# DenDen047/AcinoSet

Measured on AMD Instinct MI355X. Metric: frames/sec to SBA convergence, 6-cam x 20-kp (points-only SBA, configs[1]), higher is better.
Workload: dtype f64; 1 GPU; sba_points C=6 frames=100/rank L=20 (configs[1]); n_points_per_rank=2000, obs_slots_per_rank=12000, parallelism=frame-shard x1

## Files before the change

acinoset_amd/_native.py:

```python
from __future__ import annotations

import ctypes as C
import os
import threading
from typing import Optional

import numpy as np

try:
    import torch
except Exception:
    torch = None

_HERE = os.path.dirname(os.path.abspath(__file__))
LIB_PATH = os.environ.get('ACINOSET_HIP_LIB', os.path.join(_HERE, 'libacinoset_hip.so'))

ACS_DEVICE_PTRS = 1
ACS_CAM_STRIDE = 20
STATUS_NAMES = ('running', 'gtol', 'ftol', 'xtol', 'stalled', 'maxiter', 'noobs')
SD_MODES = {'const': 0, 'variable': 1}

SYMBOLS = (
    'acs_ctx_create', 'acs_ctx_destroy', 'acs_last_error', 'acs_ctx_set_stream', 'acs_ctx_sync',
    'acs_abi_version', 'acs_device_count', 'acs_sba_default_opts', 'acs_project_fisheye',
    'acs_sba_residuals', 'acs_sba_points', 'acs_sba_points_dense', 'acs_redescending_loss', 'acs_fk',
    'acs_fte_default_opts', 'acs_fte_solve', 'acs_fte_eval', 'acs_triangulate_pairs', 'acs_triangulate_dense',
    'acs_sba_ext_default_opts', 'acs_sba_extrinsics', 'acs_sba_points_dense_io',
    'acs_fte_dist_create', 'acs_fte_dist_init', 'acs_fte_dist_round', 'acs_fte_dist_poll',
    'acs_fte_dist_gather', 'acs_fte_dist_scatter', 'acs_fte_dist_result',
    'acs_fte_dist_destroy', 'acs_fte_dist_reset', 'acs_alloc_events', 'acs_ekf_singular_count',
    'acs_fte_debug_blocks', 'acs_fte_debug_plan',
    'acs_sba_ext_dist_create', 'acs_sba_ext_dist_init', 'acs_sba_ext_dist_round', 'acs_sba_ext_dist_poll',
    'acs_sba_ext_dist_result', 'acs_sba_ext_dist_destroy', 'acs_ekf_run',
    'acs_sba_ekf_pipeline', 'acs_fte_covariance',
)


class NativeUnavailable(RuntimeError):
    pass


class SbaOpts(C.Structure):
    _fields_ = [('max_iters', C.c_int32), ('reserved', C.c_int32), ('f_scale', C.c_double),
                ('ftol', C.c_double), ('xtol', C.c_double), ('gtol', C.c_double)]


class Report(C.Structure):
    _fields_ = [('n_problems', C.c_int64), ('status_counts', C.c_int64 * 7), ('iters_max', C.c_int64),
                ('iters_sum', C.c_int64), ('nfev_sum', C.c_int64), ('cost_before', C.c_double),
                ('cost_after', C.c_double)]

    def as_dict(self):
        return dict(n_problems=self.n_problems,
                    status_counts={STATUS_NAMES[i]: int(self.status_counts[i]) for i in range(7)},
                    iters_max=self.iters_max, iters_sum=self.iters_sum, nfev_sum=self.nfev_sum,
                    cost_before=self.cost_before, cost_after=self.cost_after)


class EkfInitSpec(C.Structure):
    _fields_ = [(k, C.c_int32) for k in ('nose', 'lure', 'x0', 'y0', 'psi0', 'xl', 'yl', 'from_sba')]


def ekf_numerics_mode(ref_numerics, jacobian):
    if jacobian == 'analytic':
        if ref_numerics:
            raise ValueError("jacobian='analytic' runs in float64: pass ref_numerics=False")
        return 2
# ... 44 lines not shown

    def as_dict(self):
        d = {k: getattr(self, k) for k, _ in self._fields_}
        d['status_name'] = STATUS_NAMES[self.status] if 0 <= self.status < 7 else str(self.status)
        return d


ABI_VERSION = 5
_lib = None
_lock = threading.Lock()
_P = C.c_void_p
_D = C.POINTER(C.c_double)


def _declare(lib):
    i32, i64, u32, dbl = C.c_int32, C.c_int64, C.c_uint32, C.c_double
    sig = {
        'acs_ctx_create': (C.c_int, [C.c_int, C.POINTER(_P)]),
        'acs_ctx_destroy': (C.c_int, [_P]),
        'acs_last_error': (C.c_char_p, [_P]),
        'acs_ctx_set_stream': (C.c_int, [_P, _P]),
        'acs_ctx_sync': (C.c_int, [_P]),
        'acs_abi_version': (C.c_int, []),
        'acs_device_count': (C.c_int, [C.POINTER(C.c_int)]),
        'acs_sba_default_opts': (None, [C.POINTER(SbaOpts)]),
        'acs_project_fisheye': (C.c_int, [_P, _P, i32, _P, _P, i64, i32, _P, u32]),
        'acs_sba_residuals': (C.c_int, [_P, _P, i32, _P, _P, _P, i64, _P, i64, _P, u32]),
        'acs_sba_points': (C.c_int, [_P, _P, i32, _P, _P, _P, i64, _P, i64, C.POINTER(SbaOpts), _P, _P,
                                     C.POINTER(Report), u32]),
        'acs_sba_points_dense': (C.c_int, [_P, _P, i32, _P, _P, i64, _P, C.POINTER(SbaOpts), C.POINTER(Report),
                                           u32]),
        'acs_sba_points_dense_io': (C.c_int, [_P, _P, i32, _P, _P, i64, _P, _P, C.POINTER(SbaOpts),
                                              C.POINTER(Report), u32]),
        'acs_redescending_loss': (C.c_int, [_P, _P, i64, dbl, dbl, dbl, _P, _P, u32]),
        'acs_fk': (C.c_int, [_P, _P, i64, _P, i64, _P, _P, _P, _P, i64, i32, i32, _P, _P, u32]),
        'acs_fte_default_opts': (None, [C.POINTER(FteOpts)]),
        'acs_fte_solve': (C.c_int, [_P, _P, i64, _P, i64, _P, i32, _P, _P, i32, i32, dbl, _P, i32, i32, _P, _P,
                                    C.POINTER(FteOpts), C.POINTER(FteReport), u32]),
        'acs_fte_eval': (C.c_int, [_P, _P, i64, _P, i64, _P, i32, _P, _P, i32, i32, dbl, _P, i32, i32, _P, _P,
                                   _P, _P, _P, u32]),
        'acs_fte_covariance': (C.c_int, [_P, _P, i64, _P, i64, _P, i32, _P, _P, i32, i32, dbl, _P, i32, i32, _P, _P,
                                         _P, _P, _P, C.POINTER(FteCovReport), u32]),
        'acs_fte_debug_blocks': (C.c_int, [_P, _P, i64, _P, i64, _P, i32, _P, _P, i32, i32, dbl, _P, i32, i32, _P, _P,
                                           dbl, i32, _P, C.POINTER(i64), u32]),
        'acs_fte_debug_plan': (C.c_int, [_P, i32, i32, i32, i32, i32, i32, C.POINTER(i32), C.POINTER(i32), i32]),
        'acs_triangulate_pairs': (C.c_int, [_P, _P, i32, _P, _P, _P, _P, i64, _P, u32]),
        'acs_triangulate_dense': (C.c_int, [_P, _P, i32, _P, _P, i64, _P, _P, u32]),
        'acs_sba_ext_default_opts': (None, [C.POINTER(SbaExtOpts)]),
        'acs_fte_dist_create': (C.c_int, [_P, _P, i64, _P, i64, _P, i32, _P, _P, i32, i32, dbl, _P, i32, i32, _P, _P,
                                          C.POINTER(FteOpts), i32, i32, C.POINTER(_P), C.POINTER(i64), u32]),
        'acs_fte_dist_init': (C.c_int, [_P, _P]),
        'acs_fte_dist_round': (C.c_int, [_P, _P, _P]),
        'acs_fte_dist_poll': (C.c_int, [_P, i64, C.POINTER(i32)]),
        'acs_fte_dist_gather': (C.c_int, [_P, _P]),
        'acs_fte_dist_scatter': (C.c_int, [_P, _P]),
        'acs_fte_dist_result': (C.c_int, [_P, _P, _P, C.POINTER(FteReport), u32]),
        'acs_fte_dist_destroy': (C.c_int, [_P]),
        'acs_fte_dist_reset': (C.c_int, [_P, _P, _P, u32]),
        'acs_alloc_events': (C.c_int64, []),
        'acs_ekf_singular_count': (C.c_int, [_P, C.POINTER(i32)]),
        'acs_sba_ext_dist_create': (C.c_int, [_P, _P, i32, _P, _P, _P, i64, _P, i64, C.POINTER(SbaExtOpts), i32, i32,
                                              C.POINTER(_P), C.POINTER(i64), u32]),
        'acs_sba_ext_dist_init': (C.c_int, [_P, _P]),
        'acs_sba_ext_dist_round': (C.c_int, [_P, _P, _P]),
        'acs_sba_ext_dist_poll': (C.c_int, [_P, C.c_int64, C.POINTER(i32)]),
        'acs_sba_ext_dist_result': (C.c_int, [_P, _P, _P, C.POINTER(SbaExtReport), u32]),
# ... 130 lines not shown
                                                int(bool(fte_form)), _ptr(out), 0), 'acs_project_fisheye')
        return out

    def sba_residuals(self, cams, uv, pt_idx, cam_idx, pts):
        cams = _c64(cams)
        uv = _c64(uv).reshape(-1, 2)
        pi = np.ascontiguousarray(pt_idx, np.int32)
        ci = np.ascontiguousarray(cam_idx, np.int32)
        pts = _c64(pts).reshape(-1, 3)
        out = np.empty(2 * len(uv))
        self.check(self.lib.acs_sba_residuals(self.h, _ptr(cams), len(cams), _ptr(uv), _ptr(pi), _ptr(ci), len(uv),
                                              _ptr(pts), len(pts), _ptr(out), 0), 'acs_sba_residuals')
        return out

    @staticmethod
    def sba_opts(f_scale=50.0, max_iters=100, ftol=1e-15, xtol=1e-9, gtol=1e-10):
        return SbaOpts(int(max_iters), 0, float(f_scale), float(ftol), float(xtol), float(gtol))

    def sba_points(self, cams, uv, pt_idx, cam_idx, pts0, opts=None, residuals=True):
        cams = _c64(cams)
        uv = _c64(uv).reshape(-1, 2)
        pi = np.ascontiguousarray(pt_idx, np.int32)
        ci = np.ascontiguousarray(cam_idx, np.int32)
        pts = _c64(pts0).reshape(-1, 3).copy()
        rb = np.empty(2 * len(uv)) if residuals else None
        ra = np.empty(2 * len(uv)) if residuals else None
        rep = Report()
        opts = opts or self.sba_opts()
        self.check(self.lib.acs_sba_points(self.h, _ptr(cams), len(cams), _ptr(uv), _ptr(pi), _ptr(ci), len(uv),
                                           _ptr(pts), len(pts), C.byref(opts), _ptr(rb), _ptr(ra), C.byref(rep), 0),
                   'acs_sba_points')
        return pts, rb, ra, rep.as_dict()

    def sba_points_dense(self, cams, uv, mask, pts0, opts=None):
        cams = _c64(cams)
        C_ = len(cams)
        uv = _c64(uv).reshape(-1, C_, 2)
        mask = np.ascontiguousarray(mask, np.uint8).reshape(-1, C_)
        pts = _c64(pts0).reshape(-1, 3).copy()
        rep = Report()
        opts = opts or self.sba_opts()
        self.check(self.lib.acs_sba_points_dense(self.h, _ptr(cams), C_, _ptr(uv), _ptr(mask), len(pts), _ptr(pts),
                                                 C.byref(opts), C.byref(rep), 0), 'acs_sba_points_dense')
        return pts, rep.as_dict()

    def sba_points_dense_dev(self, cams_p, n_cams, uv_p, mask_p, n_pts, pts_p, opts=None, report=False,
                             pts_in_p=None):
        opts = opts or self.sba_opts()
        rep = Report() if report else None
        rp = C.byref(rep) if rep is not None else None
        if pts_in_p is None:
            rc = self.lib.acs_sba_points_dense(self.h, C.c_void_p(cams_p), n_cams, C.c_void_p(uv_p),
                                               C.c_void_p(mask_p), n_pts, C.c_void_p(pts_p), C.byref(opts), rp,
                                               ACS_DEVICE_PTRS)
        else:
            rc = self.lib.acs_sba_points_dense_io(self.h, C.c_void_p(cams_p), n_cams, C.c_void_p(uv_p),
                                                  C.c_void_p(mask_p), n_pts, C.c_void_p(pts_in_p),
                                                  C.c_void_p(pts_p), C.byref(opts), rp, ACS_DEVICE_PTRS)
        self.check(rc, 'acs_sba_points_dense')
        return rep.as_dict() if rep is not None else None

    def sba_ext_opts(self, **kw):
        o = SbaExtOpts()
        self.lib.acs_sba_ext_default_opts(C.byref(o))
        for k, v in kw.items():
            setattr(o, k, v)
# ... 286 lines not shown
```

acinoset_amd/build.py:

```python
import glob
import os
import subprocess
import sys
from concurrent.futures import ThreadPoolExecutor

HERE = os.path.dirname(os.path.abspath(__file__))
REPO = os.path.dirname(HERE)
CSRC = os.path.join(HERE, 'csrc')
OUT = os.path.join(HERE, 'libacinoset_hip.so')
HIPCC = os.environ.get('HIPCC', '/opt/rocm/bin/hipcc')
ARCH = 'gfx950'
CFLAGS = ['-O3', '-std=c++17', '-fPIC', f'--offload-arch={ARCH}', '-I', os.path.join(REPO, 'include'),
          '-Wno-unused-result']


def _newest(paths):
    return max(os.path.getmtime(p) for p in paths)


def build(force: bool = False, verbose: bool = True, jobs: int = 8) -> str:
    srcs = sorted(glob.glob(os.path.join(CSRC, '*.hip')))
    deps = srcs + glob.glob(os.path.join(CSRC, '*.hpp')) + [os.path.join(REPO, 'include', 'acinoset_hip.h')]
    if not force and os.path.exists(OUT) and os.path.getmtime(OUT) >= _newest(deps):
        return OUT
    objdir = os.path.join(CSRC, 'build')
    os.makedirs(objdir, exist_ok=True)
    hdr_t = _newest([d for d in deps if not d.endswith('.hip')])

    def compile_one(src):
        obj = os.path.join(objdir, os.path.basename(src)[:-4] + '.o')
        if not force and os.path.exists(obj) and os.path.getmtime(obj) >= max(os.path.getmtime(src), hdr_t):
            return obj
        cmd = [HIPCC, *CFLAGS, '-c', src, '-o', obj]
        if verbose:
            print(' '.join(cmd), flush=True)
        subprocess.run(cmd, check=True)
        return obj

    with ThreadPoolExecutor(max_workers=jobs) as ex:
        objs = list(ex.map(compile_one, srcs))
    cmd = [HIPCC, f'--offload-arch={ARCH}', '-shared', '-fPIC', *objs, '-o', OUT]
    if verbose:
        print(' '.join(cmd), flush=True)
    subprocess.run(cmd, check=True)
    return OUT


if __name__ == '__main__':
    build(force='--force' in sys.argv)
```

acinoset_amd/csrc/common.hpp:

```cpp
#pragma once

#include <hip/hip_runtime.h>

#include <cmath>
#include <cstdarg>
#include <cstdint>
#include <cstdio>
#include <cstring>
#include <string>
#include <vector>

#include "acinoset_hip.h"

enum WsSlot {
  WS_CAMS = 0, WS_UV, WS_MASK, WS_CAMID, WS_PTS, WS_PTIDX, WS_CAMIDX, WS_OUT0, WS_OUT1,
  WS_PERPT_F0, WS_PERPT_F1, WS_PERPT_I, WS_REPORT, WS_SORT0, WS_SORT1, WS_SORT2, WS_SORT3,
  WS_TMP0, WS_TMP1, WS_TMP2, WS_TMP3, WS_TMP4, WS_TMP5, WS_TMP6, WS_TMP7,
  WS_FTE0, WS_FTE1, WS_FTE2, WS_FTE3, WS_FTE4, WS_FTE5, WS_FTE6, WS_FTE7, WS_FTE8, WS_FTE9,
  WS_FTE10, WS_FTE11, WS_FTE12, WS_FTE13, WS_FTE14, WS_FTE15,
  WS_PIPE0, WS_PIPE1, WS_PIPE2, WS_PIPE3, WS_PIPE4, WS_PIPE5, WS_PIPE6, WS_PIPE7,
  WS_NSLOTS
};
struct acs_ctx {
  int device = 0;
  hipStream_t own_stream = nullptr;
  hipStream_t stream = nullptr;
  std::string err;
  void* ws[WS_NSLOTS] = {};
  size_t ws_bytes[WS_NSLOTS] = {};
  int n_cu = 256;
  void* pinned = nullptr;
  size_t pinned_bytes = 0;
  int* ekf_bad = nullptr;
  void* fte_cov = nullptr;
  size_t fte_cov_bytes = 0;
};

hipError_t acs_dev_malloc(void** p, size_t bytes);
hipError_t acs_dev_free(void* p);
hipError_t acs_host_malloc(void** p, size_t bytes, unsigned flags);
hipError_t acs_host_free(void* p);

void* acs_pinned(acs_ctx* ctx, size_t bytes);

int acs_fail(acs_ctx* ctx, int code, const char* fmt, ...);

struct DeviceGuard {
  int prev = -1;
  explicit DeviceGuard(int device) {
    if (device < 0) return;
    if (hipGetDevice(&prev) != hipSuccess) prev = -1;
    if (prev != device) (void)hipSetDevice(device);
  }
  DeviceGuard(const DeviceGuard&) = delete;
  DeviceGuard& operator=(const DeviceGuard&) = delete;
  ~DeviceGuard() {
    int cur = -1;
    if (prev >= 0 && hipGetDevice(&cur) == hipSuccess && cur != prev) (void)hipSetDevice(prev);
  }
};
#define ACS_DEVICE_GUARD(ctx) DeviceGuard _acs_dev_guard((ctx) ? (ctx)->device : -1)

#define ACS_HIP(ctx, call)                                                                 \
  do {                                                                                     \
    hipError_t _e = (call);                                                                \
    if (_e != hipSuccess)                                                                  \
      return acs_fail((ctx), ACS_E_HIP, "%s failed: %s (%s:%d)", #call, hipGetErrorString(_e), \
                      __FILE__, __LINE__);                                                 \
// ... 153 lines not shown
  const double q1 = a * (c - E) * icb;
  const double q2 = -a * icb;
  const double K4 = K3 + 0.5 * a * cb;
  LossOut o;
  o.f = (1.0 - sa) * 0.5 * E * E + (sa - sb) * lin + (sb - sc) * q + sc * K4;
  const double dE = -0.5 * da * E * E + (1.0 - sa) * E + (da - db) * lin + (sa - sb) * a +
                    (db - dc) * q + (sb - sc) * q1 + dc * K4;
  const double ddE = -0.5 * dda * E * E - 2.0 * da * E + (1.0 - sa) + (dda - ddb) * lin +
                     2.0 * (da - db) * a + (ddb - ddc) * q + 2.0 * (db - dc) * q1 + (sb - sc) * q2 +
                     ddc * K4;
  const double sg = err > 0.0 ? 1.0 : (err < 0.0 ? -1.0 : 0.0);
  o.d1 = dE * sg;
  o.d2 = ddE;
  return o;
}

template <int CTRL>
__device__ __forceinline__ double dpp_f64(double v) {
  const int lo = __builtin_amdgcn_mov_dpp(__double2loint(v), CTRL, 0xF, 0xF, false);
  const int hi = __builtin_amdgcn_mov_dpp(__double2hiint(v), CTRL, 0xF, 0xF, false);
  return __hiloint2double(hi, lo);
}

template <int G>
__device__ __forceinline__ double group_sum(double v) {
  if (G >= 2) v += dpp_f64<0xB1>(v);
  if (G >= 4) v += dpp_f64<0x4E>(v);
  if (G >= 8) v += dpp_f64<0x141>(v);
  if (G >= 16) v += dpp_f64<0x140>(v);
  if (G >= 32) v += __shfl_xor(v, 16, G);
  if (G >= 64) v += __shfl_xor(v, 32, G);
  return v;
}
```

acinoset_amd/csrc/sba.hip:

```cpp
#include <hipcub/hipcub.hpp>

#include "common.hpp"

template <int G, int K>
__device__ __forceinline__ double group_partner(double v) {
  if constexpr (K == 0) return dpp_f64<0xB1>(v);
  else if constexpr (K == 1) return dpp_f64<0x4E>(v);
  else if constexpr (K == 2) return dpp_f64<0x141>(v);
  else if constexpr (K == 3) return dpp_f64<0x140>(v);
  else return __shfl_xor(v, 1 << K, G);
}
template <int G, int K = 0>
__device__ __forceinline__ void group_sum10(double (&v)[10], double (&p)[9]) {
  constexpr bool last = (2 << K) == G;
#pragma unroll
  for (int i = 0; i < 10; ++i) {
    const double q = group_partner<G, K>(v[i]);
    if (last && i < 9)
      p[i] = q;
    else
      v[i] += q;
  }
  if constexpr (!last) group_sum10<G, K + 1>(v, p);
}

struct SbaParams {
  int max_iters;
  double f_scale, ftol, xtol, gtol;
};

template <int G, int S, bool CAMID, bool HOIST>
__global__ __launch_bounds__(256) void k_sba_lm(const double* __restrict__ cams, int C, int K,
                                                const double2* __restrict__ uv,
                                                const uint8_t* __restrict__ mask,
                                                const uint8_t* __restrict__ camid, int64_t n_pts,
                                                const double* pts_in, double* pts,
                                                SbaParams prm,
                                                double* __restrict__ cost0, double* __restrict__ cost1,
                                                int* __restrict__ stat) {
  extern __shared__ double s_cam[];
  const unsigned bdim = blockDim.x;
  asm volatile("" ::"s"(cams), "s"(uv), "s"(mask), "s"(pts_in), "s"(n_pts), "s"(C), "s"(K), "s"(bdim));
  const int lane = threadIdx.x & (G - 1);
  const int64_t p = ((int64_t)blockIdx.x * bdim + threadIdx.x) / G;
  const bool live = p < n_pts;
  double2 q[S];
  uint8_t mk[S], cid[S];
#pragma unroll
  for (int s = 0; s < S; ++s) {
    const int slot = lane + s * G;
    q[s] = double2{0.0, 0.0};
    mk[s] = 0;
    cid[s] = (uint8_t)slot;
    if (live && slot < K) {
      const int64_t o = p * K + slot;
      mk[s] = mask[o];
      q[s] = uv[o];
      if (CAMID) cid[s] = camid[o];
    }
  }
  double x0 = 0.0, x1 = 0.0, x2 = 0.0;
  if (live) {
    x0 = pts_in[3 * p];
    x1 = pts_in[3 * p + 1];
    x2 = pts_in[3 * p + 2];
  }
  double cr[HOIST ? S : 1][ACS_CAM_STRIDE];
  if constexpr (HOIST) {
    const double* cg = cams + (size_t)(lane < C ? lane : C - 1) * ACS_CAM_STRIDE;
#pragma unroll
    for (int i = 0; i < ACS_CAM_STRIDE; ++i) cr[0][i] = cg[i];
    if (!live) return;
  } else {
    for (int i = threadIdx.x; i < C * ACS_CAM_STRIDE; i += blockDim.x) s_cam[i] = cams[i];
// ... 62 lines not shown
      const double zu = r[0] * r[0] * if2, zv = r[1] * r[1] * if2;
      const double t = zu + zv + zu * zv, u1 = 1.0 + t, ru = rcp_nr(u1);
      if constexpr (S == 1) {
        Fl = log1p_pos_ur(t, u1, ru);
      } else {
        Tl = s == 0 ? t : fma(Tl, t, Tl + t);
        rTl = s == 0 ? ru : rTl * ru;
      }
#pragma unroll
      for (int d = 0; d < 2; ++d) {
        const double z = d ? zv : zu;
        const double w = (d ? 1.0 + zu : 1.0 + zv) * ru;
        const double wh = fmax((1.0 - z) * w * w, 0.1 * w);
        const double j0 = J[3 * d], j1 = J[3 * d + 1], j2 = J[3 * d + 2];
        const double hj0 = wh * j0, hj1 = wh * j1, hj2 = wh * j2;
        Ho[0] += hj0 * j0;
        Ho[1] += hj0 * j1;
        Ho[2] += hj0 * j2;
        Ho[3] += hj1 * j1;
        Ho[4] += hj1 * j2;
        Ho[5] += hj2 * j2;
        const double wr = w * r[d];
        go[0] += wr * j0;
        go[1] += wr * j1;
        go[2] += wr * j2;
      }
    }
    if constexpr (S > 1) Fl = log1p_pos_ur(Tl, 1.0 + Tl, rTl);
#pragma unroll
    for (int i = 0; i < 6; ++i) v[i] = Ho[i];
#pragma unroll
    for (int i = 0; i < 3; ++i) v[6 + i] = go[i];
    v[9] = Fl;
    group_sum10<G>(v, vp);
    Fo = 0.5 * f2 * v[9];
    asm("" : "+v"(Fo));
  };

  double H[6], g[3], F;
  {
    double v[10], vp[9];
    linearize(x0, x1, x2, v, vp, F);
#pragma unroll
    for (int i = 0; i < 6; ++i) H[i] = v[i] + vp[i];
#pragma unroll
    for (int i = 0; i < 3; ++i) g[i] = v[6 + i] + vp[6 + i];
  }
  const double F_before = F;
  double lam = 1e-3;
  int status = ACS_STATUS_RUNNING, iters = 0, nfev = 1;
  while (true) {
    const double gmax = fmax(fabs(g[0]), fmax(fabs(g[1]), fabs(g[2])));
    const double xx = x0 * x0 + x1 * x1 + x2 * x2;
    double xs = prm.xtol + xx * rsq_nr(fmax(xx, 2.2250738585072014e-308));
    asm volatile("" : "+v"(xs));
    const double dl = 1.0 + lam;
    const double a00 = H[0] * dl, a11 = H[3] * dl, a22 = H[5] * dl;
    const double i00 = rsq_nr(a00);
    const double L10 = H[1] * i00, L20 = H[2] * i00;
    const double d11 = a11 - L10 * L10;
    const double i11 = rsq_nr(d11);
    const double L21 = (H[4] - L20 * L10) * i11;
    const double d22 = a22 - L20 * L20 - L21 * L21;
    const double i22 = rsq_nr(d22);
    const bool pd = a00 > 0.0 && d11 > 0.0 && d22 > 0.0;
    const double y0 = -g[0] * i00;
    const double y1 = (-g[1] - L10 * y0) * i11;
    const double y2 = (-g[2] - L20 * y0 - L21 * y1) * i22;
    double dx2 = y2 * i22;
    double dx1 = (y1 - L21 * dx2) * i11;
    double dx0 = (y0 - L10 * dx1 - L20 * dx2) * i00;
    asm volatile("" : "+v"(dx0), "+v"(dx1), "+v"(dx2));
    const double pred = 0.5 * (dx0 * (lam * H[0] * dx0 - g[0]) + dx1 * (lam * H[3] * dx1 - g[1]) +
                               dx2 * (lam * H[5] * dx2 - g[2]));
    if ((iters >= max_iters) | (gmax <= prm.gtol) | (pd & (pred <= ACS_COST_RES * F))) break;
    ++iters;
    const double n0 = x0 + dx0, n1 = x1 + dx1, n2 = x2 + dx2;
    double vn[10], vq[9], Fn;
    linearize(n0, n1, n2, vn, vq, Fn);
    nfev += pd ? 1 : 0;
    const double xb = prm.xtol * xs;
    const bool small = pd && dx0 * dx0 + dx1 * dx1 + dx2 * dx2 <= xb * xb;
    const bool acc = pd && Fn < F;
    const bool fconv = acc && (F - Fn) <= prm.ftol * F;
    lam = acc ? fmax(lam * 0.1, 1e-15) : lam * 10.0;
    {
      const unsigned long long am = __ballot(acc);
      unsigned long long sv;
      asm("s_and_saveexec_b64 %[sv], %[am]\n\t"
          "v_mov_b64 %[x0], %[n0]\n\tv_mov_b64 %[x1], %[n1]\n\tv_mov_b64 %[x2], %[n2]\n\t"
          "v_mov_b64 %[F], %[Fn]\n\t"
          "v_add_f64 %[h0], %[a0], %[b0]\n\tv_add_f64 %[h1], %[a1], %[b1]\n\t"
          "v_add_f64 %[h2], %[a2], %[b2]\n\tv_add_f64 %[h3], %[a3], %[b3]\n\t"
          "v_add_f64 %[h4], %[a4], %[b4]\n\tv_add_f64 %[h5], %[a5], %[b5]\n\t"
          "v_add_f64 %[g0], %[a6], %[b6]\n\tv_add_f64 %[g1], %[a7], %[b7]\n\t"
          "v_add_f64 %[g2], %[a8], %[b8]\n\t"
          "s_mov_b64 exec, %[sv]"
          : [x0] "+v"(x0), [x1] "+v"(x1), [x2] "+v"(x2), [F] "+v"(F), [h0] "+v"(H[0]), [h1] "+v"(H[1]),
            [h2] "+v"(H[2]), [h3] "+v"(H[3]), [h4] "+v"(H[4]), [h5] "+v"(H[5]), [g0] "+v"(g[0]), [g1] "+v"(g[1]),
            [g2] "+v"(g[2]), [sv] "=&s"(sv)
          : [am] "s"(am), [n0] "v"(n0), [n1] "v"(n1), [n2] "v"(n2), [Fn] "v"(Fn), [a0] "v"(vn[0]), [a1] "v"(vn[1]),
            [a2] "v"(vn[2]), [a3] "v"(vn[3]), [a4] "v"(vn[4]), [a5] "v"(vn[5]), [a6] "v"(vn[6]), [a7] "v"(vn[7]),
            [a8] "v"(vn[8]), [b0] "v"(vq[0]), [b1] "v"(vq[1]), [b2] "v"(vq[2]), [b3] "v"(vq[3]), [b4] "v"(vq[4]),
            [b5] "v"(vq[5]), [b6] "v"(vq[6]), [b7] "v"(vq[7]), [b8] "v"(vq[8])
          : "scc");
    }
    status = lam > 1e16 ? ACS_STATUS_STALLED : ACS_STATUS_RUNNING;
    status = small ? ACS_STATUS_XTOL : status;
    status = fconv ? ACS_STATUS_FTOL : status;
    if (status != ACS_STATUS_RUNNING) break;
  }
  if (status == ACS_STATUS_RUNNING) {
    const double gmax = fmax(fabs(g[0]), fmax(fabs(g[1]), fabs(g[2])));
    status = iters >= max_iters ? ACS_STATUS_MAXITER : gmax <= prm.gtol ? ACS_STATUS_GTOL : ACS_STATUS_FTOL;
  }
  if (lane == 0) {
    pts[3 * p] = x0;
    pts[3 * p + 1] = x1;
    pts[3 * p + 2] = x2;
// ... 93 lines not shown
                                                       const double* __restrict__ uvobs,
                                                       const int32_t* __restrict__ pt_idx,
                                                       const int32_t* __restrict__ cam_idx, int64_t n_obs,
                                                       const double* __restrict__ pts, int64_t n_pts,
                                                       double* __restrict__ res) {
  int64_t i = (int64_t)blockIdx.x * blockDim.x + threadIdx.x;
  if (i >= n_obs) return;
  const int c = cam_idx[i];
  const int64_t p = pt_idx[i];
  if (c < 0 || c >= n_cams || p < 0 || p >= n_pts) {
    res[2 * i] = res[2 * i + 1] = __builtin_nan("");
    return;
  }
  ProjOut o;
  fisheye_project<false>(cams + c * ACS_CAM_STRIDE, pts[3 * p], pts[3 * p + 1], pts[3 * p + 2], o);
  res[2 * i] = o.u - uvobs[2 * i];
  res[2 * i + 1] = o.v - uvobs[2 * i + 1];
}

static int next_pow2(int v) {
  int g = 1;
  while (g < v) g <<= 1;
  return g;
}

template <int G, int S, bool CAMID>
static void launch_lm_t(acs_ctx* ctx, int blocks, int block, const double* cams, int C, int K, const double2* uv,
                        const uint8_t* mask, const uint8_t* camid, int64_t n_pts, const double* pts_in, double* pts,
                        SbaParams prm, double* c0, double* c1, int* st) {
  const int64_t waves = (n_pts * G + 63) / 64;
  const bool hoist = S == 1 && !CAMID && G <= 16 && waves <= 8 * (int64_t)ctx->n_cu;
  if constexpr (S == 1 && !CAMID && G <= 16) {
    if (hoist) {
      hipLaunchKernelGGL((k_sba_lm<G, S, CAMID, true>), dim3(blocks), dim3(block),
                         sizeof(double) * ACS_CAM_STRIDE * (C + 1), ctx->stream, cams, C, K, uv, mask, camid, n_pts, pts_in,
                         pts, prm, c0, c1, st);
      return;
    }
  }
  hipLaunchKernelGGL((k_sba_lm<G, S, CAMID, false>), dim3(blocks), dim3(block), sizeof(double) * ACS_CAM_STRIDE * (C + 1),
                     ctx->stream, cams, C, K, uv, mask, camid, n_pts, pts_in, pts, prm, c0, c1, st);
}

template <int S, bool CAMID>
static int launch_lm_g(acs_ctx* ctx, int G, int blocks, int block, const double* cams, int C, int K,
                       const double2* uv, const uint8_t* mask, const uint8_t* camid, int64_t n_pts,
                       const double* pts_in, double* pts, SbaParams prm, double* c0, double* c1, int* st) {
  switch (G) {
#define ACS_G(g)                                                                                      \
  case g:                                                                                             \
    launch_lm_t<g, S, CAMID>(ctx, blocks, block, cams, C, K, uv, mask, camid, n_pts, pts_in, pts, prm, c0, c1, st); \
    break;
    ACS_G(2) ACS_G(4) ACS_G(8) ACS_G(16) ACS_G(32) ACS_G(64)
#undef ACS_G
    default:
      return acs_fail(ctx, ACS_E_INVALID, "unsupported group size %d", G);
  }
  return ACS_OK;
}

static int run_lm(acs_ctx* ctx, const double* dcams, int C, int K, const double2* duv, const uint8_t* dmask,
                  const uint8_t* dcamid, int64_t n_pts, const double* dpts_in, double* dpts,
                  const acs_sba_opts* opts, bool report, double** c0_out,
                  double** c1_out, int** st_out) {
  acs_sba_opts o;
  acs_sba_default_opts(&o);
  if (opts) o = *opts;
  ACS_CHECK(ctx, o.f_scale > 0 && o.max_iters >= 0, "bad acs_sba_opts");
  ACS_CHECK(ctx, K >= 1 && K <= 256, "observations per point (%d) must be in [1, 256]", K);
  ACS_CHECK(ctx, C >= 1 && C <= 255, "n_cams (%d) must be in [1, 255]", C);
  SbaParams prm{o.max_iters, o.f_scale, o.ftol, o.xtol, o.gtol};
  double *c0 = nullptr, *c1 = nullptr;
  int* st = nullptr;
  if (report) {
    c0 = (double*)acs_ws(ctx, WS_PERPT_F0, sizeof(double) * n_pts);
    c1 = (double*)acs_ws(ctx, WS_PERPT_F1, sizeof(double) * n_pts);
    st = (int*)acs_ws(ctx, WS_PERPT_I, sizeof(int) * 3 * n_pts);
    if (!c0 || !c1 || !st) return ACS_E_NOMEM;
  }
  int G = next_pow2(K < 2 ? 2 : K);
  int S = 1;
  if (G > 64) {
    G = 64;
    S = 4;
  } else if (G > K && (int64_t)((n_pts * G + 63) / 64) > 16 * (int64_t)ctx->n_cu) {
    const int g3 = next_pow2((K + 2) / 3);
    if (3 * g3 < G) {
      G = g3 < 2 ? 2 : g3;
      S = 3;
    }
  }
  const int64_t threads = n_pts * G;
  int block = 256;
  if (threads < (int64_t)256 * 2 * ctx->n_cu) block = 64;
  const int blocks = acs_grid(threads, block);
  int rc;
  if (dcamid) {
    rc = (S == 1) ? launch_lm_g<1, true>(ctx, G, blocks, block, dcams, C, K, duv, dmask, dcamid, n_pts, dpts_in, dpts, prm,
                                         c0, c1, st)
         : (S == 3) ? launch_lm_g<3, true>(ctx, G, blocks, block, dcams, C, K, duv, dmask, dcamid, n_pts, dpts_in, dpts,
                                           prm, c0, c1, st)
                    : launch_lm_g<4, true>(ctx, G, blocks, block, dcams, C, K, duv, dmask, dcamid, n_pts, dpts_in, dpts,
                                           prm, c0, c1, st);
  } else {
    rc = (S == 1) ? launch_lm_g<1, false>(ctx, G, blocks, block, dcams, C, K, duv, dmask, dcamid, n_pts, dpts_in, dpts,
                                          prm, c0, c1, st)
         : (S == 3) ? launch_lm_g<3, false>(ctx, G, blocks, block, dcams, C, K, duv, dmask, dcamid, n_pts, dpts_in,
                                            dpts, prm, c0, c1, st)
                    : launch_lm_g<4, false>(ctx, G, blocks, block, dcams, C, K, duv, dmask, dcamid, n_pts, dpts_in,
                                            dpts, prm, c0, c1, st);
  }
// ... 52 lines not shown
  void* tmp = acs_ws(ctx, WS_SORT3, tb);
  if (!tmp) return ACS_E_NOMEM;
  ACS_HIP(ctx, hipcub::DeviceRadixSort::SortPairs(tmp, tb, dpi, skey, (const int32_t*)vin, sval,
                                                   (int)n_obs, 0, 32, s));
  ACS_HIP(ctx, hipMemsetAsync(cnt, 0, sizeof(int32_t) * (n_pts + 2), s));
  hipLaunchKernelGGL(k_count, dim3(acs_grid(n_obs, 256)), dim3(256), 0, s, dpi, n_obs, cnt, n_pts,
                     cnt + n_pts + 1);
  ACS_HIP(ctx, hipcub::DeviceScan::ExclusiveSum(tmp, tb, cnt, start, (int)n_pts, s));
  ACS_HIP(ctx, hipcub::DeviceReduce::Max(tmp, tb, cnt, cnt + n_pts, (int)n_pts, s));
  int32_t hk[2] = {0, 0};
  ACS_HIP(ctx, hipMemcpyAsync(hk, cnt + n_pts, sizeof(int32_t) * 2, hipMemcpyDeviceToHost, s));
  ACS_HIP(ctx, hipStreamSynchronize(s));
  ACS_CHECK(ctx, hk[1] == 0, "acs_sba_points: %d point indices out of [0, %lld)", hk[1], (long long)n_pts);
  const int K = hk[0] < 1 ? 1 : hk[0];
  ACS_CHECK(ctx, K <= 256, "acs_sba_points: a point has %d observations (max 256)", K);
  double2* uvp = (double2*)acs_ws(ctx, WS_TMP2, sizeof(double2) * n_pts * K);
  uint8_t* mk = (uint8_t*)acs_ws(ctx, WS_TMP3, (size_t)n_pts * K);
  uint8_t* cid = (uint8_t*)acs_ws(ctx, WS_TMP4, (size_t)n_pts * K);
  if (!uvp || !mk || !cid) return ACS_E_NOMEM;
  ACS_HIP(ctx, hipMemsetAsync(mk, 0, (size_t)n_pts * K, s));
  hipLaunchKernelGGL(k_scatter_slots, dim3(acs_grid(n_obs, 256)), dim3(256), 0, s, skey, sval, n_obs, start,
                     (const double2*)duv, dci, K, n_cams, uvp, mk, cid);
  ACS_HIP(ctx, hipGetLastError());

  *uv_pad = uvp;
  *mask = mk;
  *camid = cid;
  *K_out = K;
  return ACS_OK;
}

extern "C" {

int acs_sba_points_dense_io(acs_ctx* ctx, const double* cams, int32_t n_cams, const double* uv,
                            const uint8_t* mask, int64_t n_pts, const double* pts_in, double* pts_out,
                            const acs_sba_opts* opts, acs_report* report, uint32_t flags) {
  ACS_DEVICE_GUARD(ctx);
  ACS_CHECK(ctx, n_pts >= 0 && n_cams >= 1 && n_cams <= 64, "acs_sba_points_dense: n_pts=%lld n_cams=%d (1..64)",
            (long long)n_pts, n_cams);
  if (n_pts == 0) {
    if (report) std::memset(report, 0, sizeof(*report));
    return ACS_OK;
  }
  void *dc, *duv, *dm, *dpi;
  int rc;
  if ((rc = acs_stage_in(ctx, WS_CAMS, cams, sizeof(double) * ACS_CAM_STRIDE * n_cams, flags, &dc))) return rc;
  if ((rc = acs_stage_in(ctx, WS_UV, uv, sizeof(double) * 2 * n_pts * n_cams, flags, &duv))) return rc;
  if ((rc = acs_stage_in(ctx, WS_MASK, mask, (size_t)n_pts * n_cams, flags, &dm))) return rc;
  if ((rc = acs_stage_in(ctx, WS_PTS, pts_in, sizeof(double) * 3 * n_pts, flags, &dpi))) return rc;
  double* dpo = (double*)acs_out_buf(ctx, WS_OUT0, pts_out, sizeof(double) * 3 * n_pts, flags);
  if (!dpo) return ACS_E_NOMEM;
  double *c0, *c1;
  int* st;
  if ((rc = run_lm(ctx, (const double*)dc, n_cams, n_cams, (const double2*)duv, (const uint8_t*)dm, nullptr, n_pts,
                   (const double*)dpi, dpo, opts, report != nullptr, &c0, &c1, &st)))
    return rc;
  if ((rc = acs_stage_out(ctx, pts_out, dpo, sizeof(double) * 3 * n_pts, flags))) return rc;
  if (report) {
    if ((rc = run_report(ctx, c0, c1, st, n_pts, report))) return rc;
  } else if (!(flags & ACS_DEVICE_PTRS)) {
    ACS_HIP(ctx, hipStreamSynchronize(ctx->stream));
  }
  return ACS_OK;
}

int acs_sba_points_dense(acs_ctx* ctx, const double* cams, int32_t n_cams, const double* uv, const uint8_t* mask,
// ... 69 lines not shown
```

include/acinoset_hip.h:

```cpp
#ifndef ACINOSET_HIP_H
#define ACINOSET_HIP_H

#include <stddef.h>
#include <stdint.h>

#ifdef __cplusplus
extern "C" {
#endif

#define ACS_ABI_VERSION 5
#define ACS_CAM_STRIDE 20

#define ACS_OK 0
#define ACS_E_INVALID -1
#define ACS_E_HIP -2
#define ACS_E_NOMEM -3
#define ACS_E_NODEV -4

#define ACS_DEVICE_PTRS 1u

#define ACS_EKF_ANALYTIC_H 2

#define ACS_STATUS_RUNNING 0
#define ACS_STATUS_GTOL 1
// ... 26 lines not shown
  double cost_before;
  double cost_after;
} acs_report;

int acs_ctx_create(int device, acs_ctx** out);
int acs_ctx_destroy(acs_ctx* ctx);
const char* acs_last_error(const acs_ctx* ctx);
int acs_ctx_set_stream(acs_ctx* ctx, void* hip_stream);
int acs_ctx_sync(acs_ctx* ctx);
int acs_abi_version(void);
int acs_device_count(int* n);
int64_t acs_alloc_events(void);
void acs_sba_default_opts(acs_sba_opts* o);

int acs_project_fisheye(acs_ctx* ctx, const double* cams, int32_t n_cams, const double* pts,
                        const int32_t* cam_idx, int64_t n, int32_t fte_form, double* uv_out,
                        uint32_t flags);

int acs_sba_residuals(acs_ctx* ctx, const double* cams, int32_t n_cams, const double* uv,
                      const int32_t* pt_idx, const int32_t* cam_idx, int64_t n_obs,
                      const double* pts, int64_t n_pts, double* resid_out, uint32_t flags);

int acs_sba_points(acs_ctx* ctx, const double* cams, int32_t n_cams, const double* uv,
                   const int32_t* pt_idx, const int32_t* cam_idx, int64_t n_obs, double* pts,
                   int64_t n_pts, const acs_sba_opts* opts, double* resid_before,
                   double* resid_after, acs_report* report, uint32_t flags);

int acs_sba_points_dense(acs_ctx* ctx, const double* cams, int32_t n_cams, const double* uv,
                         const uint8_t* mask, int64_t n_pts, double* pts,
                         const acs_sba_opts* opts, acs_report* report, uint32_t flags);
int acs_sba_points_dense_io(acs_ctx* ctx, const double* cams, int32_t n_cams, const double* uv,
                            const uint8_t* mask, int64_t n_pts, const double* pts_in, double* pts_out,
                            const acs_sba_opts* opts, acs_report* report, uint32_t flags);

int acs_redescending_loss(acs_ctx* ctx, const double* err, int64_t n, double a, double b, double c,
                          double* out, double* dout , uint32_t flags);

int acs_fk(acs_ctx* ctx, const int32_t* skel_ints, int64_t n_ints, const double* skel_reals,
           int64_t n_reals, const double* x, const double* dx, const double* ddx, const double* tau,
           int64_t n, int32_t intermode, int32_t directions, double* out, double* jac,
           uint32_t flags);

typedef struct {
  int32_t max_iters;
  int32_t window;
  double ftol;
  double xtol;
  double gtol;
  double lambda0;
  double redesc_a, redesc_b, redesc_c;
} acs_fte_opts;

typedef struct {
  int32_t status;
  int32_t iters;
  int32_t n_accepted;
  int32_t n_bad_pivots;
  double cost_before, cost_after, cost_meas, cost_model;
  double grad_max, lambda_final;
} acs_fte_report;

void acs_fte_default_opts(acs_fte_opts* o);
int acs_fte_solve(acs_ctx* ctx, const int32_t* skel_ints, int64_t n_ints, const double* skel_reals,
                  int64_t n_reals, const double* cams, int32_t n_cams, const double* meas,
                  const double* w, int32_t n_frames, int32_t shutter_delay, double Ts,
                  const double* qinv, int32_t sd_mode, int32_t intermode, double* X, double* tau,
// ... 111 lines not shown
```

Measured before the change: 12.05 million frames/s.

## Add row-broadcast DPP reduction layout for small SBA point LM kernels

Adds a 'row' LM layout for the points-only SBA kernel. Each point uses a 16-lane row with one observation slot per lane, and the per-point Hessian, gradient and cost sums are reduced with v_mov/v_fmac DPP row_newbcast instructions instead of the butterfly group_sum. The accept step folds those sums into the masked exec block. Auto mode picks this path when the point count fits within about 4 waves per CU and there are 3 to 8 observation slots. The change also fixes the hoisted blocks at 64 threads, reorders the kernel arguments, and enables kernarg preload for sba.hip. The hand-written inline asm adds correctness risk (exec masking, the DPP row semantics) and wastes lanes when K is smaller than 16.

```diff
diff --git a/acinoset_amd/_native.py b/acinoset_amd/_native.py
--- a/acinoset_amd/_native.py
+++ b/acinoset_amd/_native.py
@@ -19,6 +19,8 @@
 ACS_CAM_STRIDE = 20
 STATUS_NAMES = ('running', 'gtol', 'ftol', 'xtol', 'stalled', 'maxiter', 'noobs')
 SD_MODES = {'const': 0, 'variable': 1}
+
+SBA_LM_LAYOUTS = {'auto': 0, 'butterfly': 1, 'row': 2}
 
 SYMBOLS = (
     'acs_ctx_create', 'acs_ctx_destroy', 'acs_last_error', 'acs_ctx_set_stream', 'acs_ctx_sync',
@@ -32,7 +34,7 @@
     'acs_fte_debug_blocks', 'acs_fte_debug_plan',
     'acs_sba_ext_dist_create', 'acs_sba_ext_dist_init', 'acs_sba_ext_dist_round', 'acs_sba_ext_dist_poll',
     'acs_sba_ext_dist_result', 'acs_sba_ext_dist_destroy', 'acs_ekf_run',
-    'acs_sba_ekf_pipeline', 'acs_fte_covariance',
+    'acs_sba_ekf_pipeline', 'acs_fte_covariance', 'acs_sba_set_lm_layout', 'acs_sba_lm_layout',
 )
 
 
@@ -143,6 +145,8 @@
                                            u32]),
         'acs_sba_points_dense_io': (C.c_int, [_P, _P, i32, _P, _P, i64, _P, _P, C.POINTER(SbaOpts),
                                               C.POINTER(Report), u32]),
+        'acs_sba_set_lm_layout': (C.c_int, [_P, i32]),
+        'acs_sba_lm_layout': (C.c_int, [_P, i32, i64, i32, C.POINTER(i32)]),
         'acs_redescending_loss': (C.c_int, [_P, _P, i64, dbl, dbl, dbl, _P, _P, u32]),
         'acs_fk': (C.c_int, [_P, _P, i64, _P, i64, _P, _P, _P, _P, i64, i32, i32, _P, _P, u32]),
         'acs_fte_default_opts': (None, [C.POINTER(FteOpts)]),
@@ -339,6 +343,16 @@
                    'acs_sba_points')
         return pts, rb, ra, rep.as_dict()
 
+    def sba_set_lm_layout(self, layout='auto'):
+        self.check(self.lib.acs_sba_set_lm_layout(self.h, SBA_LM_LAYOUTS[layout]), 'acs_sba_set_lm_layout')
+
+    def sba_lm_layout(self, n_slots, n_pts, cam_ids=False):
+        n_cu = C.c_int32(0)
+        rc = self.lib.acs_sba_lm_layout(self.h, int(n_slots), int(n_pts), int(bool(cam_ids)), C.byref(n_cu))
+        if rc < 0:
+            raise ValueError('acs_sba_lm_layout: bad arguments')
+        return {v: k for k, v in SBA_LM_LAYOUTS.items()}[rc], int(n_cu.value)
+
     def sba_points_dense(self, cams, uv, mask, pts0, opts=None):
         cams = _c64(cams)
         C_ = len(cams)
diff --git a/acinoset_amd/build.py b/acinoset_amd/build.py
--- a/acinoset_amd/build.py
+++ b/acinoset_amd/build.py
@@ -12,6 +12,7 @@
 ARCH = 'gfx950'
 CFLAGS = ['-O3', '-std=c++17', '-fPIC', f'--offload-arch={ARCH}', '-I', os.path.join(REPO, 'include'),
           '-Wno-unused-result']
+FILE_CFLAGS = {'sba.hip': ['-mllvm', '-amdgpu-kernarg-preload-count=16']}
 
 
 def _newest(paths):
@@ -31,7 +32,7 @@
         obj = os.path.join(objdir, os.path.basename(src)[:-4] + '.o')
         if not force and os.path.exists(obj) and os.path.getmtime(obj) >= max(os.path.getmtime(src), hdr_t):
             return obj
-        cmd = [HIPCC, *CFLAGS, '-c', src, '-o', obj]
+        cmd = [HIPCC, *CFLAGS, *FILE_CFLAGS.get(os.path.basename(src), []), '-c', src, '-o', obj]
         if verbose:
             print(' '.join(cmd), flush=True)
         subprocess.run(cmd, check=True)
diff --git a/acinoset_amd/csrc/common.hpp b/acinoset_amd/csrc/common.hpp
--- a/acinoset_amd/csrc/common.hpp
+++ b/acinoset_amd/csrc/common.hpp
@@ -34,6 +34,7 @@
   int* ekf_bad = nullptr;
   void* fte_cov = nullptr;
   size_t fte_cov_bytes = 0;
+  int sba_lm_layout = ACS_SBA_LM_AUTO;
 };
 
 hipError_t acs_dev_malloc(void** p, size_t bytes);
@@ -253,3 +254,73 @@
   if (G >= 64) v += __shfl_xor(v, 32, G);
   return v;
 }
+
+#define ACS_ROW_BC(n) " row_newbcast:" #n " row_mask:0xf bank_mask:0xf\n\t"
+#define ACS_ROW_MOV(d, s, n) "v_mov_b64_dpp %[" #d "], %[" #s "]" ACS_ROW_BC(n)
+#define ACS_ROW_FMAC(d, s, n) "v_fmac_f64_dpp %[" #d "], %[" #s "], %[one]" ACS_ROW_BC(n)
+#define ACS_ROW_ADD(d, a, b) "v_add_f64 %[" #d "], %[" #a "], %[" #b "]\n\t"
+#define ACS_ROW_ADDT(d, t, n) ACS_ROW_ADD(d, d, t)
+#define ACS_ROW9(OP, d, s, n)                                                                             \
+  OP(d##0, s##0, n) OP(d##1, s##1, n) OP(d##2, s##2, n) OP(d##3, s##3, n) OP(d##4, s##4, n) OP(d##5, s##5, n) \
+      OP(d##6, s##6, n) OP(d##7, s##7, n) OP(d##8, s##8, n)
+#define ACS_ROW_SUMS2 ACS_ROW9(ACS_ROW_MOV, h, s, 0) ACS_ROW9(ACS_ROW_FMAC, h, s, 2)
+#define ACS_ROW_SUMS3 ACS_ROW_SUMS2 ACS_ROW9(ACS_ROW_FMAC, h, s, 4)
+#define ACS_ROW_SUMS4                                                                                \
+  ACS_ROW9(ACS_ROW_MOV, h, s, 0) ACS_ROW9(ACS_ROW_MOV, t, s, 4) ACS_ROW9(ACS_ROW_FMAC, h, s, 2)      \
+  ACS_ROW9(ACS_ROW_FMAC, t, s, 6) ACS_ROW9(ACS_ROW_ADDT, h, t, 0)
+#define ACS_ROW_H(c)                                                                                       \
+  [h0] c(H[0]), [h1] c(H[1]), [h2] c(H[2]), [h3] c(H[3]), [h4] c(H[4]), [h5] c(H[5]), [h6] c(g[0]), [h7] c(g[1]), \
+      [h8] c(g[2])
+#define ACS_ROW_T                                                                                              \
+  [t0] "=&v"(t[0]), [t1] "=&v"(t[1]), [t2] "=&v"(t[2]), [t3] "=&v"(t[3]), [t4] "=&v"(t[4]), [t5] "=&v"(t[5]), \
+      [t6] "=&v"(t[6]), [t7] "=&v"(t[7]), [t8] "=&v"(t[8])
+#define ACS_ROW_S                                                                                          \
+  [s0] "v"(s[0]), [s1] "v"(s[1]), [s2] "v"(s[2]), [s3] "v"(s[3]), [s4] "v"(s[4]), [s5] "v"(s[5]), [s6] "v"(s[6]), \
+      [s7] "v"(s[7]), [s8] "v"(s[8]), [one] "v"(one)
+
+template <int ROW>
+__device__ __forceinline__ double row_pairs_cost(double (&s)[10], const double (&q)[10], double one) {
+  double c, c2;
+#define ACS_ROW_PAIR(i) "v_add_f64 %[s" #i "], %[s" #i "], %[q" #i "]\n\t"
+#define ACS_ROW_PAIR_OPS                                                                                       \
+  [s0] "+v"(s[0]), [s1] "+v"(s[1]), [s2] "+v"(s[2]), [s3] "+v"(s[3]), [s4] "+v"(s[4]), [s5] "+v"(s[5]),          \
+      [s6] "+v"(s[6]), [s7] "+v"(s[7]), [s8] "+v"(s[8]), [s9] "+v"(s[9])
+#define ACS_ROW_PAIR_IN                                                                                        \
+  [q0] "v"(q[0]), [q1] "v"(q[1]), [q2] "v"(q[2]), [q3] "v"(q[3]), [q4] "v"(q[4]), [q5] "v"(q[5]), [q6] "v"(q[6]), \
+      [q7] "v"(q[7]), [q8] "v"(q[8]), [q9] "v"(q[9]), [one] "v"(one)
+  if constexpr (ROW == 2) {
+    asm(ACS_ROW_PAIR(9) ACS_ROW_PAIR(0) ACS_ROW_PAIR(1) ACS_ROW_MOV(c, s9, 0) ACS_ROW_PAIR(2) ACS_ROW_PAIR(3)
+            ACS_ROW_FMAC(c, s9, 2) ACS_ROW_PAIR(4) ACS_ROW_PAIR(5) ACS_ROW_PAIR(6) ACS_ROW_PAIR(7) ACS_ROW_PAIR(8)
+        : [c] "=&v"(c), ACS_ROW_PAIR_OPS
+        : ACS_ROW_PAIR_IN);
+  } else if constexpr (ROW == 3) {
+    asm(ACS_ROW_PAIR(9) ACS_ROW_PAIR(0) ACS_ROW_PAIR(1) ACS_ROW_MOV(c, s9, 0) ACS_ROW_PAIR(2) ACS_ROW_PAIR(3)
+            ACS_ROW_FMAC(c, s9, 2) ACS_ROW_PAIR(4) ACS_ROW_PAIR(5) ACS_ROW_FMAC(c, s9, 4) ACS_ROW_PAIR(6)
+                ACS_ROW_PAIR(7) ACS_ROW_PAIR(8)
+        : [c] "=&v"(c), ACS_ROW_PAIR_OPS
+        : ACS_ROW_PAIR_IN);
+  } else {
+    static_assert(ROW == 4, "row-broadcast sums are written out for 2, 3 and 4 lane pairs");
+    asm(ACS_ROW_PAIR(9) ACS_ROW_PAIR(0) ACS_ROW_PAIR(1) ACS_ROW_MOV(c, s9, 0) ACS_ROW_MOV(c2, s9, 4) ACS_ROW_PAIR(2)
+            ACS_ROW_FMAC(c, s9, 2) ACS_ROW_FMAC(c2, s9, 6) ACS_ROW_PAIR(3) ACS_ROW_PAIR(4) ACS_ROW_ADD(c, c, c2)
+                ACS_ROW_PAIR(5) ACS_ROW_PAIR(6) ACS_ROW_PAIR(7) ACS_ROW_PAIR(8)
+        : [c] "=&v"(c), [c2] "=&v"(c2), ACS_ROW_PAIR_OPS
+        : ACS_ROW_PAIR_IN);
+  }
+#undef ACS_ROW_PAIR
+#undef ACS_ROW_PAIR_OPS
+#undef ACS_ROW_PAIR_IN
+  return c;
+}
+
+template <int ROW>
+__device__ __forceinline__ void row_sums9(double (&H)[6], double (&g)[3], const double (&s)[10], double one) {
+  if constexpr (ROW == 2) {
+    asm(ACS_ROW_SUMS2 : ACS_ROW_H("=&v") : ACS_ROW_S);
+  } else if constexpr (ROW == 3) {
+    asm(ACS_ROW_SUMS3 : ACS_ROW_H("=&v") : ACS_ROW_S);
+  } else {
+    double t[9];
+    asm(ACS_ROW_SUMS4 : ACS_ROW_H("=&v"), ACS_ROW_T : ACS_ROW_S);
+  }
+}
diff --git a/acinoset_amd/csrc/sba.hip b/acinoset_amd/csrc/sba.hip
--- a/acinoset_amd/csrc/sba.hip
+++ b/acinoset_amd/csrc/sba.hip
@@ -29,17 +29,18 @@
   double f_scale, ftol, xtol, gtol;
 };
 
-template <int G, int S, bool CAMID, bool HOIST>
-__global__ __launch_bounds__(256) void k_sba_lm(const double* __restrict__ cams, int C, int K,
-                                                const double2* __restrict__ uv,
-                                                const uint8_t* __restrict__ mask,
-                                                const uint8_t* __restrict__ camid, int64_t n_pts,
-                                                const double* pts_in, double* pts,
+template <int G, int S, bool CAMID, bool HOIST, int ROW = 0>
+__global__ __launch_bounds__(256) void k_sba_lm(const double2* __restrict__ uv,
+                                                const uint8_t* __restrict__ mask, int64_t n_pts,
+                                                const double* pts_in, const double* __restrict__ cams,
+                                                int K, int C, const uint8_t* __restrict__ camid,
+                                                double* pts,
                                                 SbaParams prm,
                                                 double* __restrict__ cost0, double* __restrict__ cost1,
                                                 int* __restrict__ stat) {
+  static_assert(ROW == 0 || (G == 16 && S == 1 && !CAMID && HOIST), "ROW: 16-lane rows, one slot per lane, hoisted records");
   extern __shared__ double s_cam[];
-  const unsigned bdim = blockDim.x;
+  const unsigned bdim = HOIST ? 64u : blockDim.x;
   asm volatile("" ::"s"(cams), "s"(uv), "s"(mask), "s"(pts_in), "s"(n_pts), "s"(C), "s"(K), "s"(bdim));
   const int lane = threadIdx.x & (G - 1);
   const int64_t p = ((int64_t)blockIdx.x * bdim + threadIdx.x) / G;
@@ -168,8 +169,15 @@
 #pragma unroll
     for (int i = 0; i < 3; ++i) v[6 + i] = go[i];
     v[9] = Fl;
-    group_sum10<G>(v, vp);
-    Fo = 0.5 * f2 * v[9];
+    if constexpr (ROW) {
+      double qp[10];
+#pragma unroll
+      for (int i = 0; i < 10; ++i) qp[i] = dpp_f64<0xB1>(v[i]);
+      Fo = 0.5 * f2 * row_pairs_cost<ROW>(v, qp, 1.0);
+    } else {
+      group_sum10<G>(v, vp);
+      Fo = 0.5 * f2 * v[9];
+    }
     asm("" : "+v"(Fo));
   };
 
@@ -177,10 +185,14 @@
   {
     double v[10], vp[9];
     linearize(x0, x1, x2, v, vp, F);
-#pragma unroll
-    for (int i = 0; i < 6; ++i) H[i] = v[i] + vp[i];
-#pragma unroll
-    for (int i = 0; i < 3; ++i) g[i] = v[6 + i] + vp[6 + i];
+    if constexpr (ROW) {
+      row_sums9<ROW>(H, g, v, 1.0);
+    } else {
+#pragma unroll
+      for (int i = 0; i < 6; ++i) H[i] = v[i] + vp[i];
+#pragma unroll
+      for (int i = 0; i < 3; ++i) g[i] = v[6 + i] + vp[6 + i];
+    }
   }
   const double F_before = F;
   double lam = 1e-3;
@@ -200,6 +212,7 @@
     const double d22 = a22 - L20 * L20 - L21 * L21;
     const double i22 = rsq_nr(d22);
     const bool pd = a00 > 0.0 && d11 > 0.0 && d22 > 0.0;
+    [[maybe_unused]] const unsigned long long pdm = ROW ? __ballot(pd) : 0ull;
     const double y0 = -g[0] * i00;
     const double y1 = (-g[1] - L10 * y0) * i11;
     const double y2 = (-g[2] - L20 * y0 - L21 * y1) * i22;
@@ -220,7 +233,28 @@
     const bool acc = pd && Fn < F;
     const bool fconv = acc && (F - Fn) <= prm.ftol * F;
     lam = acc ? fmax(lam * 0.1, 1e-15) : lam * 10.0;
-    {
+    if constexpr (ROW) {
+      const unsigned long long am = __builtin_amdgcn_ballot_w64(Fn < F) & pdm;
+      unsigned long long sv;
+      const double one = 1.0;
+      const double(&s)[10] = vn;
+#define ACS_ROW_ACCEPT(SUMS, ...)                                                                          \
+  asm("s_and_saveexec_b64 %[sv], %[am]\n\t"                                                                \
+      "v_mov_b64 %[x0], %[n0]\n\tv_mov_b64 %[x1], %[n1]\n\tv_mov_b64 %[x2], %[n2]\n\t"                    \
+      "v_mov_b64 %[F], %[Fn]\n\t" SUMS "s_mov_b64 exec, %[sv]"                                             \
+      : [x0] "+v"(x0), [x1] "+v"(x1), [x2] "+v"(x2), [F] "+v"(F), ACS_ROW_H("+v"), [sv] "=&s"(sv) __VA_ARGS__ \
+      : [am] "s"(am), [n0] "v"(n0), [n1] "v"(n1), [n2] "v"(n2), [Fn] "v"(Fn), ACS_ROW_S                    \
+      : "scc")
+      if constexpr (ROW == 2) {
+        ACS_ROW_ACCEPT(ACS_ROW_SUMS2);
+      } else if constexpr (ROW == 3) {
+        ACS_ROW_ACCEPT(ACS_ROW_SUMS3);
+      } else {
+        double t[9];
+        ACS_ROW_ACCEPT(ACS_ROW_SUMS4, , ACS_ROW_T);
+      }
+#undef ACS_ROW_ACCEPT
+    } else {
       const unsigned long long am = __ballot(acc);
       unsigned long long sv;
       asm("s_and_saveexec_b64 %[sv], %[am]\n\t"
@@ -380,14 +414,16 @@
   const bool hoist = S == 1 && !CAMID && G <= 16 && waves <= 8 * (int64_t)ctx->n_cu;
   if constexpr (S == 1 && !CAMID && G <= 16) {
     if (hoist) {
+      block = 64;
+      blocks = acs_grid(n_pts * G, block);
       hipLaunchKernelGGL((k_sba_lm<G, S, CAMID, true>), dim3(blocks), dim3(block),
-                         sizeof(double) * ACS_CAM_STRIDE * (C + 1), ctx->stream, cams, C, K, uv, mask, camid, n_pts, pts_in,
+                         sizeof(double) * ACS_CAM_STRIDE * (C + 1), ctx->stream, uv, mask, n_pts, pts_in, cams, K, C, camid,
                          pts, prm, c0, c1, st);
       return;
     }
   }
   hipLaunchKernelGGL((k_sba_lm<G, S, CAMID, false>), dim3(blocks), dim3(block), sizeof(double) * ACS_CAM_STRIDE * (C + 1),
-                     ctx->stream, cams, C, K, uv, mask, camid, n_pts, pts_in, pts, prm, c0, c1, st);
+                     ctx->stream, uv, mask, n_pts, pts_in, cams, K, C, camid, pts, prm, c0, c1, st);
 }
 
 template <int S, bool CAMID>
@@ -405,6 +441,29 @@
       return acs_fail(ctx, ACS_E_INVALID, "unsupported group size %d", G);
   }
   return ACS_OK;
+}
+
+static bool lm_row_selected(const acs_ctx* ctx, int K, int64_t n_pts, bool camid) {
+  const bool legal = !camid && K >= 3 && K <= 8;
+  if (!legal || ctx->sba_lm_layout == ACS_SBA_LM_BUTTERFLY) return false;
+  if (ctx->sba_lm_layout == ACS_SBA_LM_ROW) return true;
+  return (n_pts * 16 + 63) / 64 <= 4 * (int64_t)ctx->n_cu;
+}
+
+static void launch_lm_row(acs_ctx* ctx, const double* cams, int C, int K, const double2* uv, const uint8_t* mask,
+                          int64_t n_pts, const double* pts_in, double* pts, SbaParams prm, double* c0, double* c1,
+                          int* st) {
+  const dim3 grid(acs_grid(n_pts * 16, 64)), block(64);
+  const size_t lds = sizeof(double) * ACS_CAM_STRIDE * (C + 1);
+#define ACS_ROW_LAUNCH(r)                                                                                        \
+  hipLaunchKernelGGL((k_sba_lm<16, 1, false, true, r>), grid, block, lds, ctx->stream, uv, mask, n_pts, pts_in, cams, \
+                     K, C, (const uint8_t*)nullptr, pts, prm, c0, c1, st)
+  switch ((K + 1) / 2) {
+    case 2: ACS_ROW_LAUNCH(2); break;
+    case 3: ACS_ROW_LAUNCH(3); break;
+    default: ACS_ROW_LAUNCH(4); break;
+  }
+#undef ACS_ROW_LAUNCH
 }
 
 static int run_lm(acs_ctx* ctx, const double* dcams, int C, int K, const double2* duv, const uint8_t* dmask,
@@ -425,6 +484,14 @@
     c1 = (double*)acs_ws(ctx, WS_PERPT_F1, sizeof(double) * n_pts);
     st = (int*)acs_ws(ctx, WS_PERPT_I, sizeof(int) * 3 * n_pts);
     if (!c0 || !c1 || !st) return ACS_E_NOMEM;
+  }
+  if (lm_row_selected(ctx, K, n_pts, dcamid != nullptr)) {
+    launch_lm_row(ctx, dcams, C, K, duv, dmask, n_pts, dpts_in, dpts, prm, c0, c1, st);
+    ACS_HIP(ctx, hipGetLastError());
+    *c0_out = c0;
+    *c1_out = c1;
+    *st_out = st;
+    return ACS_OK;
   }
   int G = next_pow2(K < 2 ? 2 : K);
   int S = 1;
@@ -543,6 +610,20 @@
 
 extern "C" {
 
+int acs_sba_set_lm_layout(acs_ctx* ctx, int32_t layout) {
+  if (!ctx) return ACS_E_INVALID;
+  ACS_CHECK(ctx, layout == ACS_SBA_LM_AUTO || layout == ACS_SBA_LM_BUTTERFLY || layout == ACS_SBA_LM_ROW,
+            "acs_sba_set_lm_layout: layout %d", layout);
+  ctx->sba_lm_layout = layout;
+  return ACS_OK;
+}
+
+int acs_sba_lm_layout(const acs_ctx* ctx, int32_t n_slots, int64_t n_pts, int32_t with_cam_ids, int32_t* n_cu) {
+  if (!ctx || n_slots < 1 || n_pts < 0) return -1;
+  if (n_cu) *n_cu = ctx->n_cu;
+  return lm_row_selected(ctx, n_slots, n_pts, with_cam_ids != 0) ? ACS_SBA_LM_ROW : ACS_SBA_LM_BUTTERFLY;
+}
+
 int acs_sba_points_dense_io(acs_ctx* ctx, const double* cams, int32_t n_cams, const double* uv,
                             const uint8_t* mask, int64_t n_pts, const double* pts_in, double* pts_out,
                             const acs_sba_opts* opts, acs_report* report, uint32_t flags) {
diff --git a/include/acinoset_hip.h b/include/acinoset_hip.h
--- a/include/acinoset_hip.h
+++ b/include/acinoset_hip.h
@@ -82,6 +82,13 @@
 int acs_sba_points_dense_io(acs_ctx* ctx, const double* cams, int32_t n_cams, const double* uv,
                             const uint8_t* mask, int64_t n_pts, const double* pts_in, double* pts_out,
                             const acs_sba_opts* opts, acs_report* report, uint32_t flags);
+
+#define ACS_SBA_LM_AUTO 0
+#define ACS_SBA_LM_BUTTERFLY 1
+#define ACS_SBA_LM_ROW 2
+int acs_sba_set_lm_layout(acs_ctx* ctx, int32_t layout);
+int acs_sba_lm_layout(const acs_ctx* ctx, int32_t n_slots, int64_t n_pts, int32_t with_cam_ids,
+                      int32_t* n_cu);
 
 int acs_redescending_loss(acs_ctx* ctx, const double* err, int64_t n, double a, double b, double c,
                           double* out, double* dout , uint32_t flags);
```

Result: faster. 12.62 million frames/s, median of 6 (+4.7%).
